# HaiminLuo/svox_t

Measured on AMD Instinct MI355X. Metric: Mrays/s fwd+bwd, 800×800 render, depth-8 SH9 N3Tree, 1→8 MI355X, higher is better.
Workload: dtype f32

## Files before the change

### svox_t_amd/csrc/svoxt_fwd_kernels.h

```cpp
#pragma once

#include <hip/hip_runtime.h>
#include <stdint.h>

#include "svoxt_device.h"
#include "svoxt_lists.h"

#pragma clang fp contract(off)

#ifndef SVOXT_ROLES_CSUM
#define SVOXT_ROLES_CSUM 1
#endif

namespace svoxt {

template <bool N2>
__device__ __forceinline__ uint32_t leaf_slot(const TreeDev& tr, const Ray& r, float t, uint32_t slot) {
    if (slot != 0xffffffffu) return slot;
    Leaf lf;
    locate<N2>(tr, r.ox + t * r.dx, r.oy + t * r.dy, r.oz + t * r.dz, lf);
    return lf.slot;
}

template <int FMT, int C, int BD, bool N2, bool REC, bool XF = false, bool RESUME = false, bool LOBES = false>
__device__ __forceinline__ void render_fwd_ray(const TreeDev& tr, const RaysDev& rays, const Opts& opt, float* __restrict__ out,
                                               const RecLists& L, uint4* __restrict__ aux, const int64_t tid) {
    static_assert(!XF || FMT == FMT_SH, "view rotations only matter for view-dependent formats");
    static_assert(!LOBES || (FMT == FMT_SH && !XF), "lobes stand in for an SH basis");
    static_assert(!(RESUME && REC), "the tail launch does not record");
    constexpr int K = (FMT == FMT_RGBA) ? (C + 1) : (C * BD + 1);
    __shared__ uint2 rstage[REC ? kRecBlock * kBlock : 1];
    __shared__ int32_t ltab[REC ? kMaxRecBlocks : 1];
    __shared__ float4 tstage[(REC && C == 3 && !XF) ? 4 * kBlock : 1];
    if constexpr (REC) rec_tab_init(ltab);
    const int S = L.S;
    int64_t cur_block = 0;
    const int64_t q = ray_of_thread(rays, tid);
    if (q >= rays.Q) return;
    float* o = out + q * (C + 1);
    float t_start = 0.f;
    if constexpr (RESUME) {
        const uint4 a = aux[q];
        if ((a.x & kRecOverflow) == 0u || a.w == kAuxStopped) return;
        t_start = __uint_as_float(a.y);
    }

    Ray r;
    if (!setup_ray(tr, rays, opt, q, r)) {
#pragma unroll
        for (int j = 0; j < C; ++j) o[j] = opt.background_brightness;
        o[C] = 0.f;
        if constexpr (REC) aux[q] = make_uint4(0u, 0u, __float_as_uint(1.f), 0u);
        return;
    }
    int nrec = 0;
    bool over = false;
    float t_resume = 0.f;
    float basis[BD > 0 ? BD : 1];
    float vd[3] = {0.f, 0.f, 0.f};
    if constexpr (FMT == FMT_SH) {
        load_vdir(rays, q, vd);
        if constexpr (LOBES) precalc_lobes<BD>(opt.format, tr, vd[0], vd[1], vd[2], basis);
        else if constexpr (!XF) precalc_basis<BD>(FMT_SH, BD, tr, vd[0], vd[1], vd[2], basis);
    }
    float acc[C];
#pragma unroll
    for (int j = 0; j < C; ++j) acc[j] = 0.f;

    float light = 1.f;
    float t = r.tmin;
    if constexpr (RESUME) {
#pragma unroll
        for (int j = 0; j < C; ++j) acc[j] = o[j];
        light = o[C];
        t = t_start;
    }
    bool stopped = false;
    auto shade = [&](const float (&row)[K], int32_t idx, float delta_t, float t_cur, uint32_t slot) -> bool {
        const float sigma = row[K - 1];
        if (!(sigma > (REC ? 0.f : opt.sigma_thresh))) return false;
        const bool comp = !REC || (sigma > opt.sigma_thresh && !stopped);
        bool recorded = false;
        if constexpr (REC) {
            bool room = nrec < S;
            if (room && (nrec & 7) == 0) {
                cur_block = rec_block_begin(L, ltab, tid >> 6, nrec >> 3);
                room = cur_block >= 0;
            }
            recorded = room;
            if (room) {
                rec_stage_put(rstage, (int)threadIdx.x, L.rec, cur_block, nrec, (uint32_t)idx, delta_t);
                ++nrec;
            } else if (!over) {
                over = true;
                t_resume = t_cur;
            }
        }
        const float att = pexpf(-delta_t * r.delta_scale * sigma);
        const float weight = light * (1.f - att);
        float ex[C];
        if constexpr (FMT == FMT_SH) {
            if constexpr (XF) rotated_sh_basis<BD>(tr, idx, vd, basis);
#pragma unroll
            for (int c = 0; c < C; ++c) {
                ex[c] = pexpf(neg_sh_dot<BD>(basis, row + c * BD));
                if (comp) acc[c] = (float)((double)acc[c] + (double)weight / (1.0 + (double)ex[c]));
            }
        } else {
#pragma unroll
            for (int j = 0; j < C; ++j) {
                ex[j] = pexpf(-row[j]);
                if (comp) acc[j] = (float)((double)acc[j] + (double)weight / (1.0 + (double)ex[j]));
            }
        }
        if constexpr (REC && C == 3 && !XF) {
            if (recorded && L.terms != nullptr) {
                const int k = nrec - 1;
                tstage[(k & 3) * kBlock + threadIdx.x] =
                    make_float4(pexpf(-delta_t * sigma * r.delta_scale), ex[0], ex[1], ex[2]);
                if ((k & 3) == 3) terms_flush(tstage, (int)threadIdx.x, L.terms, cur_block, k);
            }
        }
        if (comp) {
            light *= att;
            if (tr.weight_accum != nullptr) atomicAdd(tr.weight_accum + leaf_slot<N2>(tr, r, t_cur, slot), weight);
            if (light <= opt.stop_thresh) {
                if constexpr (!REC) return true;
                stopped = true;
            }
        }
        return false;
    };
    Sample s;
    bool have = t < r.tmax;
    if (have) march_step<N2>(tr, r, opt.step_size, t, s);
    while (have) {
        float row[K];
        const bool valid = s.valid;
        if (valid) load_row<K>(tr.features + (int64_t)s.idx * K, row);
        const float t_cur = t, delta_t = s.delta_t;
        const int32_t idx = s.idx;
        const uint32_t slot = s.leaf.slot;
        t = march_advance(t, delta_t);
        have = t < r.tmax;
        if (have) march_step<N2>(tr, r, opt.step_size, t, s);
        if (valid && shade(row, idx, delta_t, t_cur, slot)) { stopped = true; break; }
    }
    if (stopped) {
        const float scale = (float)(1.0 / (1.0 - (double)light));
#pragma unroll
        for (int j = 0; j < C; ++j) o[j] = acc[j] * scale;
    } else {
        const float bg = light * opt.background_brightness;
#pragma unroll
        for (int j = 0; j < C; ++j) o[j] = acc[j] + bg;
    }
    o[C] = 1.f - light;
    if constexpr (REC) {
        rec_stage_finish(rstage, (int)threadIdx.x, L.rec, cur_block, nrec);
        if constexpr (C == 3 && !XF) {
            if (L.terms != nullptr && (nrec & 3)) terms_flush(tstage, (int)threadIdx.x, L.terms, cur_block, nrec - 1);
        }
        aux[q] = make_uint4((uint32_t)nrec | (over ? kRecOverflow : 0u), __float_as_uint(t_resume),
                            __float_as_uint(light), 0u);
        if (over) note_overflow(L);
    }
    if constexpr (RESUME) aux[q].z = __float_as_uint(light);
}

template <int FMT, int C, int BD, bool N2, bool REC, bool XF = false, bool RESUME = false, bool LOBES = false>
__global__ void __launch_bounds__(kBlock)
render_fwd_kernel(TreeDev tr, RaysDev rays, Opts opt, float* __restrict__ out,
                  RecLists L, uint4* __restrict__ aux) {
    if constexpr (RESUME) {
        if (no_ray_overflowed(L)) return;
    }
    render_fwd_ray<FMT, C, BD, N2, REC, XF, RESUME, LOBES>(tr, rays, opt, out, L, aux,
                                                           ((int64_t)blockIdx.x + rays.tile0) * kBlock + threadIdx.x);
}

template <bool N2>
__global__ void __launch_bounds__(kBlock)
render_fwd_generic_kernel(TreeDev tr, RaysDev rays, Opts opt, int C, float* __restrict__ out) {
    const int64_t q = ray_of_thread(rays, (int64_t)blockIdx.x * kBlock + threadIdx.x);
    if (q >= rays.Q) return;
    float* o = out + q * (C + 1);
    const int K = tr.K;

    Ray r;
    if (!setup_ray(tr, rays, opt, q, r)) {
        for (int j = 0; j < C; ++j) o[j] = opt.background_brightness;
        o[C] = 0.f;
        return;
    }
    for (int j = 0; j < C; ++j) o[j] = 0.f;
    float basis[25];
    float vd[3];
    load_vdir(rays, q, vd);
    precalc_basis<0>(opt.format, opt.basis_dim, tr, vd[0], vd[1], vd[2], basis);
    float light = 1.f;
    float t = r.tmin;
    while (t < r.tmax) {
        Sample s;
        march_step<N2>(tr, r, opt.step_size, t, s);
        if (s.valid) {
            const float* row = tr.features + (int64_t)s.idx * K;
            const float sigma = row[K - 1];
            if (sigma > opt.sigma_thresh) {
                const float att = pexpf(-s.delta_t * r.delta_scale * sigma);
                const float weight = light * (1.f - att);
                if (tr.xform != nullptr) rotated_basis(tr, opt.format, opt.basis_dim, s.idx, vd, basis);
                if (opt.format != FMT_RGBA) {
                    for (int c = 0; c < C; ++c) {
                        const int off = c * opt.basis_dim;
                        float tmp = 0.f;
                        for (int i = opt.min_comp; i <= opt.max_comp; ++i) tmp += basis[i] * row[off + i];
                        o[c] = (float)((double)o[c] + (double)weight / (1.0 + (double)pexpf(-tmp)));
                    }
                } else {
                    for (int j = 0; j < C; ++j)
                        o[j] = (float)((double)o[j] + (double)weight / (1.0 + (double)pexpf(-row[j])));
                }
                light *= att;
                if (tr.weight_accum != nullptr) atomicAdd(tr.weight_accum + leaf_slot<N2>(tr, r, t, s.leaf.slot), weight);
                if (light <= opt.stop_thresh) {
                    const float scale = (float)(1.0 / (1.0 - (double)light));
                    for (int j = 0; j < C; ++j) o[j] *= scale;
                    o[C] = 1.f - light;
                    return;
                }
            }
        }
        t = march_advance(t, s.delta_t);
    }
    for (int j = 0; j < C; ++j) o[j] += light * opt.background_brightness;
    o[C] = 1.f - light;
}


__global__ void __launch_bounds__(256)
sigma_mask_kernel(const float* __restrict__ features, int64_t M, int K, float thresh, unsigned long long* __restrict__ mask,
                  unsigned mask_blocks = ~0u, uint4* __restrict__ fill = nullptr, int64_t fill_vec = 0) {
    if (blockIdx.x >= mask_blocks) {
        const int64_t i0 = ((int64_t)(blockIdx.x - mask_blocks) * 256 + threadIdx.x) * 4;
#pragma unroll
        for (int j = 0; j < 4; ++j)
            if (i0 + j < fill_vec) fill[i0 + j] = make_uint4(~0u, ~0u, ~0u, ~0u);
        return;
    }
    const int lane = threadIdx.x & 63;
    const int64_t word0 = ((int64_t)blockIdx.x * 4 + (threadIdx.x >> 6)) * 4;
    const int64_t words = (M + 63) / 64;
    float v[4];
#pragma unroll
    for (int j = 0; j < 4; ++j) {
        const int64_t row = (word0 + j) * 64 + lane;
        v[j] = row < M ? features[row * K + (K - 1)] : thresh;
    }
#pragma unroll
    for (int j = 0; j < 4; ++j) {
        const unsigned long long b = __ballot(v[j] > thresh);
        if (lane == j && word0 + j < words) mask[word0 + j] = b;
    }
}

template <int K>
__global__ void __launch_bounds__(256)
exp_table_kernel(const float* __restrict__ features, int64_t M, float thresh, uint8_t* __restrict__ mask_bytes,
                 float* __restrict__ etab) {
    static_assert(K == 8 || K == 16 || K == 32, "row widths with a table");
    constexpr int P = K / 4, RW = 64 / P;
    typedef float v4f __attribute__((ext_vector_type(4)));
    const int64_t t = (int64_t)blockIdx.x * 256 + threadIdx.x;
    const int64_t row = t / P;
    const int part = (int)(t % P);
    bool bit = false;
    if (row < M) {
        const v4f v = __builtin_nontemporal_load(reinterpret_cast<const v4f*>(features) + t);
        v4f e;
        e.x = pexpf(-v.x); e.y = pexpf(-v.y); e.z = pexpf(-v.z);
        if (part == P - 1) { e.w = v.w; bit = v.w > thresh; }
        else e.w = pexpf(-v.w);
        reinterpret_cast<v4f*>(etab)[t] = e;
    }
    const unsigned long long b = __ballot(bit);
    if (mask_bytes != nullptr && (threadIdx.x & 63) == 0 && row < M) {
        uint32_t bits = 0u;
#pragma unroll
        for (int i = 0; i < RW; ++i) bits |= (uint32_t)((b >> (i * P + P - 1)) & 1ull) << i;
        uint8_t* dst = mask_bytes + (row >> 3);
#pragma unroll
        for (int j = 0; j < RW / 8; ++j) dst[j] = (uint8_t)(bits >> (8 * j));
    }
}

template <bool N2, bool STOP, int ACC, bool MASK, bool CSUM = false>
__device__ __forceinline__ uint32_t march_rec_tile(const TreeDev& tr, const RaysDev& rays, const Opts& opt, const RecLists& L,
                                                   uint4* __restrict__ aux, const uint32_t* __restrict__ sigma_mask,
                                                   int64_t tile, uint2* __restrict__ rstage, int32_t* __restrict__ ltab,
                                                   uint32_t* csum = nullptr) {
    static_assert(!(MASK && STOP), "the stop rule needs sigma itself");
    const int lane = (int)(threadIdx.x & 63);
    uint32_t cs = 0u;
    if (csum != nullptr) *csum = 0u;
    rec_tab_init(ltab);
    const int S = L.S;
    int64_t cur_block = 0;
    const int64_t tid = tile * 64 + lane;
    const int64_t q = ray_of_thread(rays, tid);
    if (q >= rays.Q) return 0u;
    Ray r;
    if (!setup_ray(tr, rays, opt, q, r)) {
        aux[q] = make_uint4(0u, 0u, __float_as_uint(1.f), 0u);
        return 0u;
    }
    const int K = tr.K;
    const float* __restrict__ sig_col = tr.features + (K - 1);
    int nrec = 0;
    uint32_t over = 0u;
    float t_resume = 0.f;
    float light = 1.f;
    float t = r.tmin;
    const float kNone = -__builtin_inff();
    float p_sigma = kNone, p_dt = 0.f, p_t = 0.f;
    int32_t p_idx = 0;
    uint32_t p_word = 0u;
    auto pending = [&]() -> bool {
        if constexpr (MASK) return ((p_word >> (p_idx & 31)) & 1u) != 0u;
        else return p_sigma > (STOP ? opt.sigma_thresh : 0.f);
    };
    while (t < r.tmax) {
        Sample s;
        march_step<N2, ACC>(tr, r, opt.step_size, t, s);
        const float t_cur = t;
        t = march_advance(t, s.delta_t);
        bool keep = true;
        if (pending()) {
            bool room = nrec < S;
            if (room && (nrec & 7) == 0) {
                cur_block = rec_block_begin(L, ltab, tid >> 6, nrec >> 3);
                room = cur_block >= 0;
            }
            if (room) {
                rec_stage_put(rstage, lane, L.rec, cur_block, nrec, (uint32_t)p_idx, p_dt);
                if constexpr (CSUM) cs ^= rec_hash(nrec, (uint32_t)p_idx, __float_as_uint(p_dt));
                ++nrec;
                if constexpr (STOP) {
                    light *= pexpf(-p_dt * r.delta_scale * p_sigma);
                    if (light <= opt.stop_thresh) { t = __builtin_inff(); keep = false; }
                }
            } else {
                over = kRecOverflow;
                t_resume = p_t;
                t = __builtin_inff();
                keep = false;
            }
        }
        p_sigma = kNone;
        p_word = 0u;
        if (keep && s.valid) {
            if constexpr (MASK) p_word = sigma_mask[s.idx >> 5];
            else p_sigma = sig_col[(int64_t)s.idx * K];
            p_idx = s.idx;
            p_dt = s.delta_t;
            p_t = t_cur;
        }
    }
    if (pending()) {
        bool room = nrec < S;
        if (room && (nrec & 7) == 0) {
            cur_block = rec_block_begin(L, ltab, tid >> 6, nrec >> 3);
            room = cur_block >= 0;
        }
        if (room) {
            rec_stage_put(rstage, lane, L.rec, cur_block, nrec, (uint32_t)p_idx, p_dt);
            if constexpr (CSUM) cs ^= rec_hash(nrec, (uint32_t)p_idx, __float_as_uint(p_dt));
            ++nrec;
        } else {
            over = kRecOverflow;
            t_resume = p_t;
        }
    }
    rec_stage_finish(rstage, lane, L.rec, cur_block, nrec);
    aux[q] = make_uint4((uint32_t)nrec | over, __float_as_uint(t_resume), __float_as_uint(1.f), 0u);
    if (over != 0u) note_overflow(L);
    if constexpr (CSUM) *csum = cs;
    return (uint32_t)nrec | over;
}

template <bool N2, bool STOP, int ACC, bool MASK = false>
__global__ void __launch_bounds__(kBlock)
march_rec_kernel(TreeDev tr, RaysDev rays, Opts opt, RecLists L, uint4* __restrict__ aux,
                 const uint32_t* __restrict__ sigma_mask = nullptr) {
    __shared__ uint2 rstage[kRecBlock * kBlock];
    __shared__ int32_t ltab[kMaxRecBlocks];
    const int64_t tile = (int64_t)blockIdx.x + rays.tile0;
    march_rec_tile<N2, STOP, ACC, MASK>(tr, rays, opt, L, aux, sigma_mask, tile, rstage, ltab);
}

constexpr int kShadeP = 7;
typedef float shade_v4f __attribute__((ext_vector_type(4)));
template <int FMT, int BD, bool XF, bool STOP, bool WTERMS, bool COH, bool LOBES = false>
__device__ __forceinline__ uint32_t shade_tile_body(const TreeDev& tr, const RaysDev& rays, const Opts& opt, const RecLists& L,
                                                    uint4* __restrict__ aux, float* __restrict__ out, int64_t tile,
                                                    shade_v4f (*terms)[kShadeP][64] ,
                                                    bool stale_test = false, uint32_t* ax_used = nullptr ) {
    constexpr int C = 3, W = 8, P = kShadeP;
    static_assert(P == W - 1, "one wavefront runs along the rays");
    constexpr int K = (FMT == FMT_RGBA) ? (C + 1) : (C * BD + 1);
    constexpr int NB = (FMT == FMT_SH) ? BD : 1;
    typedef shade_v4f v4f;
    const int lane = threadIdx.x & 63, wave = threadIdx.x >> 6;
    const int64_t q = ray_of_thread(rays, tile * 64 + lane);
    const bool inb = q < rays.Q;
    uint32_t a_x = 0u;
    if (inb) a_x = COH ? aux_get_coherent(aux + q).x : aux[q].x;
    int nrec = (int)(a_x & ~kRecOverflow);
    if constexpr (COH) {
        nrec = min(nrec, L.S);
        if (ax_used != nullptr) *ax_used = a_x;
    }
    int maxn = nrec;
    for (int off = 32; off > 0; off >>= 1) maxn = max(maxn, __shfl_xor(maxn, off, 64));
    maxn = __builtin_amdgcn_readfirstlane(maxn);
    const int nround = (maxn + P - 1) / P;
    const int32_t tabreg = rec_tab_reg<COH>(L, tile, lane);
    uint32_t cs = 0u;

    float delta_scale = 0.f;
    float basis[NB];
    float vd[3] = {0.f, 0.f, 0.f};
    if (wave > 0 && nrec > 0) {
        Ray r;
        setup_ray(tr, rays, opt, q, r);
        delta_scale = r.delta_scale;
        if constexpr (FMT == FMT_SH) {
            load_vdir(rays, q, vd);
            if constexpr (LOBES) precalc_lobes<BD>(opt.format, tr, vd[0], vd[1], vd[2], basis);
            else if constexpr (!XF) precalc_basis<BD>(FMT_SH, BD, tr, vd[0], vd[1], vd[2], basis);
        }
    }
    float light = 1.f, acc[C] = {0.f, 0.f, 0.f};
    bool stopped = false;

    for (int rd = 0; rd <= nround; ++rd) {
        if (wave > 0) {
            const int k = rd * P + (wave - 1);
            if (rd < nround && k < nrec) {
                int64_t blk = rec_block_u(L, tabreg, tile, k >> 3);
                if constexpr (COH) blk = min(max(blk, (int64_t)0), L.pool_blocks - 1);
                uint2 e = COH ? rec_get_coherent(L.rec + rec_index_in(blk, lane, k)) : rec_get(L.rec + rec_index_in(blk, lane, k));
                if constexpr (COH) {
                    if (stale_test && k == 0) e.x ^= 1u;
                    if constexpr (SVOXT_ROLES_CSUM != 0) cs ^= rec_hash(k, e.x, e.y);
                    e.x = min(e.x, (uint32_t)(tr.M - 1));
                }
                const int32_t idx = (int32_t)e.x;
                float row[K];
                load_row<K>(tr.features + (int64_t)idx * K, row);
                v4f tv;
                tv.x = pexpf(-__uint_as_float(e.y) * delta_scale * row[K - 1]);
                const bool below = !(row[K - 1] > opt.sigma_thresh);
                if constexpr (FMT == FMT_SH) {
                    if constexpr (XF) rotated_sh_basis<BD>(tr, idx, vd, basis);
                    float ex[C];
#pragma unroll
                    for (int c = 0; c < C; ++c) {
                        ex[c] = pexpf(neg_sh_dot<BD>(basis, row + c * BD));
                    }
                    tv.y = ex[0]; tv.z = ex[1]; tv.w = ex[2];
                } else {
                    tv.y = pexpf(-row[0]); tv.z = pexpf(-row[1]); tv.w = pexpf(-row[2]);
                }
                {
                    v4f tl = tv;
                    tl.x = below ? 1.f : tv.x;
                    terms[rd & 1][wave - 1][lane] = tl;
                }
                if constexpr (WTERMS) {
                    typedef float v4g __attribute__((ext_vector_type(4)));
                    const float att_b = pexpf(-__uint_as_float(e.y) * row[K - 1] * delta_scale);
                    __builtin_nontemporal_store(v4g{att_b, tv.y, tv.z, tv.w},
                                                reinterpret_cast<v4g*>(L.terms + terms_index_pm(blk, lane, k)));
                }
            }
        } else if (rd > 0) {
            const int kb = (rd - 1) * P;
#pragma unroll
            for (int j = 0; j < P; ++j) {
                if (kb + j < nrec && !stopped) {
                    const v4f tv = terms[(rd - 1) & 1][j][lane];
                    const float weight = light * (1.f - tv.x);
                    acc[0] = (float)((double)acc[0] + (double)weight / (1.0 + (double)tv.y));
                    acc[1] = (float)((double)acc[1] + (double)weight / (1.0 + (double)tv.z));
                    acc[2] = (float)((double)acc[2] + (double)weight / (1.0 + (double)tv.w));
                    light *= tv.x;
                    if (light <= opt.stop_thresh) stopped = true;
                }
            }
        }
        lds_barrier();
    }
    if (wave == 0 && inb) {
        uint32_t* aw = reinterpret_cast<uint32_t*>(aux + q);
        float* o = out + q * (C + 1);
        if (stopped) {
            const float scale = (float)(1.0 / (1.0 - (double)light));
#pragma unroll
            for (int j = 0; j < C; ++j) o[j] = acc[j] * scale;
            o[C] = 1.f - light;
            if constexpr (STOP) aw[0] = a_x & ~kRecOverflow;
        } else if (a_x & kRecOverflow) {
#pragma unroll
            for (int j = 0; j < C; ++j) o[j] = acc[j];
            o[C] = light;
        } else {
            const float bg = light * opt.background_brightness;
#pragma unroll
            for (int j = 0; j < C; ++j) o[j] = acc[j] + bg;
            o[C] = 1.f - light;
        }
        aw[2] = __float_as_uint(light);
        if constexpr (!STOP) aw[3] = stopped ? kAuxStopped : 0u;
    }
    return cs;
}

constexpr int kRolePolls = 20000;
constexpr int64_t kTileEmpty = 1 << 30;
__device__ __forceinline__ int my_xcc() { return (int)(__builtin_amdgcn_s_getreg((3 << 11) | 20) & (kRoleXcds - 1)); }
enum { kRoleCtrShaded = 256, kRoleCtrMismatch = 257, kRoleCtrGaveUp = 258, kRoleCtrDropped = 259, kRoleCtrFallback = 260 };
enum { kRoleTestDrop = 1, kRoleTestNoPoll = 2, kRoleTestStale = 4, kRoleAgentFence = 8 };

constexpr int32_t kTileShaded = 0x200;
template <int FMT, int BD, bool XF, bool STOP, bool WTERMS = false, bool LOBES = false>
__global__ void __launch_bounds__(512)
shade_tile_kernel(TreeDev tr, RaysDev rays, Opts opt, RecLists L,
                  uint4* __restrict__ aux, float* __restrict__ out, const int32_t* __restrict__ tile_state = nullptr) {
    static_assert(!LOBES || (FMT == FMT_SH && !XF), "lobes stand in for an SH basis");
    __shared__ shade_v4f terms[2][kShadeP][64];
    const int64_t tile = (int64_t)blockIdx.x + rays.tile0;
    if (tile_state != nullptr && tile_state[tile] == kTileShaded) return;
    shade_tile_body<FMT, BD, XF, STOP, WTERMS, false, LOBES>(tr, rays, opt, L, aux, out, tile, terms);
    if (tile_state != nullptr && threadIdx.x == 0)
        atomicAdd(const_cast<int32_t*>(tile_state) + roles_even(gridDim.x + rays.tile0) + kRoleCtrFallback, 1);
}

template <int FMT, int BD, bool WTERMS, bool LOBES = false, bool XF = false>
__global__ void __launch_bounds__(512)
fwd_finish_kernel(TreeDev tr, RaysDev rays, Opts opt, RecLists L, uint4* __restrict__ aux, float* __restrict__ out,
                  int32_t* __restrict__ tile_state, int ntiles) {
    __shared__ shade_v4f terms[2][kShadeP][64];
    constexpr int CAP = 64;
    __shared__ int32_t s_list[CAP];
    __shared__ int32_t s_n;
    const int run = (ntiles + (int)gridDim.x - 1) / (int)gridDim.x;
    const int t0 = (int)blockIdx.x * run, t1 = min(t0 + run, ntiles);
    if (t0 >= t1) return;
    if (threadIdx.x == 0) s_n = 0;
    __syncthreads();
    for (int i = t0 + (int)threadIdx.x; i < t1; i += 512) {
        if (tile_state[i] != kTileShaded) {
            const int pos = atomicAdd(&s_n, 1);
            if (pos < CAP) s_list[pos] = i;
        }
    }
    __syncthreads();
    const int n = s_n;
    int32_t* const fallback_ctr = tile_state + roles_even(ntiles) + kRoleCtrFallback;
    if (n > CAP) {
        for (int tile = t0; tile < t1; ++tile) {
            if (tile_state[tile] == kTileShaded) continue;
            shade_tile_body<FMT, BD, XF, false, WTERMS, false, LOBES>(tr, rays, opt, L, aux, out, tile, terms);
            if (threadIdx.x == 0) atomicAdd(fallback_ctr, 1);
            __syncthreads();
        }
    } else {
        for (int j = 0; j < n; ++j) {
            shade_tile_body<FMT, BD, XF, false, WTERMS, false, LOBES>(tr, rays, opt, L, aux, out, s_list[j], terms);
            if (threadIdx.x == 0) atomicAdd(fallback_ctr, 1);
            __syncthreads();
        }
    }
    if (no_ray_overflowed(L)) return;
    __syncthreads();
    for (int tile = t0 + (int)(threadIdx.x >> 6); tile < t1; tile += 8)
        render_fwd_ray<FMT, 3, BD, true, false, XF, true, LOBES>(tr, rays, opt, out, L, aux, (int64_t)tile * 64 + (threadIdx.x & 63));
}

__device__ __forceinline__ void publish_tile(int32_t* __restrict__ tile_state, int ntiles, int64_t tile, uint32_t csum,
                                             bool agent_fence) {
    asm volatile("s_waitcnt vmcnt(0)" ::: "memory");
    if (agent_fence) {
        __builtin_amdgcn_fence(__ATOMIC_RELEASE, "agent");
        asm volatile("s_waitcnt vmcnt(0)" ::: "memory");
    }
    if ((threadIdx.x & 63) == 0) {
        const int xcc = my_xcc();
        const int64_t base = roles_even(ntiles);
        int32_t* ctr = tile_state + base + xcc * 32;
        unsigned long long* queue = reinterpret_cast<unsigned long long*>(tile_state + base + 16 * 32) + (int64_t)xcc * ntiles;
        const int pos = __hip_atomic_fetch_add(ctr, 1, __ATOMIC_RELAXED, __HIP_MEMORY_SCOPE_AGENT) + 1;
        __hip_atomic_store(queue + pos, (unsigned long long)(uint32_t)tile | ((unsigned long long)csum << 32), __ATOMIC_RELAXED,
                           __HIP_MEMORY_SCOPE_AGENT);
    }
}
__device__ __forceinline__ unsigned long long pop_tile(int32_t* __restrict__ tile_state, int ntiles, int polls) {
    const int xcc = my_xcc();
    const int64_t base = roles_even(ntiles);
    int32_t* ctr = tile_state + base + xcc * 32;
    unsigned long long* queue = reinterpret_cast<unsigned long long*>(tile_state + base + 16 * 32) + (int64_t)xcc * ntiles;
    unsigned long long ent = ~0ull;
    const int idx = __hip_atomic_fetch_add(ctr + 16, 1, __ATOMIC_RELAXED, __HIP_MEMORY_SCOPE_AGENT) + 1;
    if (idx < ntiles) {
        for (int p = 0; p < polls; ++p) {
            ent = __hip_atomic_load(queue + idx, __ATOMIC_RELAXED, __HIP_MEMORY_SCOPE_AGENT);
            if (ent != ~0ull) break;
            __builtin_amdgcn_s_sleep(16);
        }
    }
    return ent;
}

struct RolesMap {
    int gb, full, gb_last;
    int cnt[8];
};
__host__ __device__ inline int64_t roles_group_of(const RolesMap& m, int b) {
    if (m.gb <= 0) return b;
    const int x = b & 7, s = b >> 3;
    if (s < m.full * m.gb) return ((int64_t)(s / m.gb) * 8 + x) * m.gb + s % m.gb;
    return (int64_t)m.full * 8 * m.gb + (int64_t)x * m.gb_last + (s - m.full * m.gb);
}

template <int FMT, int BD, int ACC, bool WTERMS, bool LOBES = false, bool XF = false>
__global__ void __launch_bounds__(512)
fwd_roles_kernel(TreeDev tr, RaysDev rays, Opts opt, RecLists L, uint4* __restrict__ aux, float* __restrict__ out,
                 const uint32_t* __restrict__ sigma_mask, int32_t* __restrict__ tile_state, int n_march, int ntiles,
                 int tflags , RolesMap map) {
    constexpr int kMarchBytes = 8 * (kRecBlock * 64 * (int)sizeof(uint2) + kMaxRecBlocks * (int)sizeof(int32_t));
    constexpr int kShadeBytes = 2 * kShadeP * 64 * (int)sizeof(shade_v4f);
    __shared__ __attribute__((aligned(16))) unsigned char lds[kMarchBytes > kShadeBytes ? kMarchBytes : kShadeBytes];
    __shared__ unsigned long long s_ent;
    const int wave = threadIdx.x >> 6;
    const bool agent_fence = (tflags & kRoleAgentFence) != 0;
    int32_t* const ctrs = tile_state + roles_even(ntiles);
    if ((int)blockIdx.x < n_march) {
        const int64_t tile = roles_group_of(map, (int)blockIdx.x) * 8 + wave;
        if (tile >= ntiles) return;
        uint2* rstage = reinterpret_cast<uint2*>(lds) + wave * (kRecBlock * 64);
        int32_t* ltab = reinterpret_cast<int32_t*>(lds + 8 * kRecBlock * 64 * sizeof(uint2)) + wave * kMaxRecBlocks;
        __builtin_amdgcn_s_setprio(3);
        uint32_t cs_lane;
        const uint32_t ax = march_rec_tile<true, false, ACC, true, SVOXT_ROLES_CSUM != 0>(tr, rays, opt, L, aux, sigma_mask, tile, rstage, ltab, &cs_lane);
        const bool empty = __ballot(ax != 0u) == 0ull;
        if (empty) {
            const int64_t q = ray_of_thread(rays, tile * 64 + (threadIdx.x & 63));
            if (q < rays.Q) {
                const float light = 1.f, acc = 0.f;
                const float bg = light * opt.background_brightness;
                float* o = out + q * 4;
                o[0] = acc + bg; o[1] = acc + bg; o[2] = acc + bg;
                o[3] = 1.f - light;
            }
            if ((threadIdx.x & 63) == 0) tile_state[tile] = kTileShaded;
        }
        uint32_t csum = 0u;
        if constexpr (SVOXT_ROLES_CSUM != 0) csum = empty ? 0u : tile_checksum(ax != 0u ? cs_lane : 0u, ax, (int)(threadIdx.x & 63));
        publish_tile(tile_state, ntiles, empty ? (tile | kTileEmpty) : tile, csum, agent_fence);
        return;
    }
    const int i = (int)blockIdx.x - n_march, a = i & 7, b = i >> 3;
    if (b >= map.cnt[a]) return;
    if (threadIdx.x == 0) s_ent = pop_tile(tile_state, ntiles, (tflags & kRoleTestNoPoll) ? 1 : kRolePolls);
    __syncthreads();
    const unsigned long long ent = s_ent;
    if (ent == ~0ull) {
        if (threadIdx.x == 0) atomicAdd(ctrs + kRoleCtrGaveUp, 1);
        return;
    }
    const int64_t tile = (int64_t)(uint32_t)ent;
    if (tile >= ntiles) return;
    if ((tflags & kRoleTestDrop) && tile % 3 == 0) {
        if (threadIdx.x == 0) atomicAdd(ctrs + kRoleCtrDropped, 1);
        return;
    }
    if (agent_fence) __builtin_amdgcn_fence(__ATOMIC_ACQUIRE, "agent");
    uint32_t ax = 0u;
    static_assert(!XF || (FMT == FMT_SH && !LOBES && BD <= 9), "view rotations: SH rows");
    const uint32_t part = shade_tile_body<FMT, BD, XF, false, WTERMS, true, LOBES>(
        tr, rays, opt, L, aux, out, tile, reinterpret_cast<shade_v4f (*)[kShadeP][64]>(lds), (tflags & kRoleTestStale) && tile % 5 == 0, &ax);
    uint32_t* s_part = reinterpret_cast<uint32_t*>(lds);
    s_part[threadIdx.x] = part;
    lds_barrier();
    if (wave == 0) {
        const int lane = (int)threadIdx.x;
        uint32_t x = 0u;
#pragma unroll
        for (int w = 0; w < 8; ++w) x ^= s_part[w * 64 + lane];
        const uint32_t c = SVOXT_ROLES_CSUM != 0 ? tile_checksum(ax != 0u ? x : 0u, ax, lane) : (uint32_t)(ent >> 32);
        if (lane == 0) {
        if (c == (uint32_t)(ent >> 32)) {
            tile_state[tile] = kTileShaded;
            atomicAdd(ctrs + kRoleCtrShaded, 1);
        } else {
            atomicAdd(ctrs + kRoleCtrMismatch, 1);
        }
        }
    }
}

#ifndef SVOXT_CHAN_SWIZZLE
#define SVOXT_CHAN_SWIZZLE 1
#endif
template <int K, bool STOP, bool FAST, bool ETAB = false>
__global__ void __launch_bounds__(256)
shade_chan_kernel(TreeDev tr, RaysDev rays, Opts opt, RecLists L,
                  uint4* __restrict__ aux, float* __restrict__ out, int keep_over = 0) {
    static_assert(K == 8 || K == 16 || K == 32, "row widths with a channel-lane instance");
    static_assert(!(ETAB && FAST), "the table holds the exact exponentials");
    constexpr int RPW = 64 / K;
    const int lane = threadIdx.x & 63;
    const int c = lane & (K - 1);
    const int sig_lane = lane | (K - 1);
    constexpr unsigned kRun = (unsigned)(K / 4) * SVOXT_CHAN_SWIZZLE;
    const unsigned b0 = blockIdx.x;
    unsigned wg = b0;
    if (kRun != 0u && (b0 | (8u * kRun - 1u)) < gridDim.x) {
        const unsigned base = b0 & ~(8u * kRun - 1u), x = b0 & 7u, m = (b0 >> 3) & (kRun - 1u);
        wg = base + x * kRun + m;
    }
    const int64_t t = (int64_t)rays.tile0 * 64 + ((int64_t)wg * (blockDim.x >> 6) + (threadIdx.x >> 6)) * RPW + (lane / K);
    const int64_t q = ray_of_thread(rays, t);
    const bool inb = q < rays.Q;
    uint4 a = make_uint4(0u, 0u, 0u, 0u);
    if (inb) a = aux[q];
    const int nrec = (int)(a.x & ~kRecOverflow);
    int maxn = nrec;
    for (int off = 32; off >= K; off >>= 1) maxn = max(maxn, __shfl_xor(maxn, off, 64));
    maxn = __builtin_amdgcn_readfirstlane(maxn);
    float ds = 0.f;
    if (nrec > 0) {
        Ray r;
        setup_ray(tr, rays, opt, q, r);
        ds = r.delta_scale;
    }
    const int32_t tabreg = rec_tab_reg(L, t >> 6, lane);
    float light = 1.f, acc = 0.f;
    bool stopped = false;
    typedef unsigned int v4u __attribute__((ext_vector_type(4)));
    const bool is_sig = c == K - 1;
    const char* __restrict__ col_base = reinterpret_cast<const char*>(ETAB ? tr.etab : tr.features) + 4 * c;
    constexpr float kNegLog2e = -1.44269504088896341f;
    const float sc_mult = is_sig ? ds * kNegLog2e : 0.f, sc_base = is_sig ? 0.f : kNegLog2e;
    for (int kb = 0; kb < maxn; kb += kRecBlock) {
        uint32_t idx[kRecBlock];
        float dt[kRecBlock], ex[kRecBlock];
        const int n_here = nrec - kb;
        const int64_t blk = rec_block_u(L, tabreg, t >> 6, kb >> 3);
        const v4u* line = reinterpret_cast<const v4u*>(L.rec + rec_index_in(blk, t, kb));
#pragma unroll
        for (int j = 0; j < kRecBlock / 2; ++j) {
            const v4u w = __builtin_nontemporal_load(line + j);
            idx[2 * j] = w.x; dt[2 * j] = __uint_as_float(w.y);
            idx[2 * j + 1] = w.z; dt[2 * j + 1] = __uint_as_float(w.w);
        }
        float x[kRecBlock];
#pragma unroll
        for (int j = 0; j < kRecBlock; ++j) {
            const uint32_t row = j < n_here ? idx[j] : 0u;
            x[j] = *reinterpret_cast<const float*>(col_base + (size_t)row * (size_t)(K * 4));
        }
        float att_mine = 1.f;
        if constexpr (ETAB) {
            const int jm = c & (kRecBlock - 1);
            float sg = 0.f, dm = 0.f;
#pragma unroll
            for (int j = 0; j < kRecBlock; ++j) {
                const float sj = __shfl(x[j], sig_lane, 64);
                sg = jm == j ? sj : sg;
                dm = jm == j ? dt[j] : dm;
            }
            att_mine = pexpf((jm < n_here && sg > opt.sigma_thresh) ? -dm * ds * sg : 0.f);
#pragma unroll
            for (int j = 0; j < kRecBlock; ++j) ex[j] = j < n_here ? x[j] : 1.f;
        } else {
#pragma unroll
        for (int j = 0; j < kRecBlock; ++j) {
            if constexpr (FAST) {
                const float e2 = x[j] * __builtin_fmaf(dt[j], sc_mult, sc_base);
                ex[j] = __builtin_amdgcn_exp2f((j < n_here && !(is_sig && !(x[j] > opt.sigma_thresh))) ? e2 : 0.f);
            } else {
                const float arg = is_sig ? ((x[j] > opt.sigma_thresh) ? -dt[j] * ds * x[j] : 0.f) : -x[j];
                ex[j] = pexpf(j < n_here ? arg : 0.f);
            }
        }
        }
#pragma unroll
        for (int j = 0; j < kRecBlock; ++j) {
            const float att = ETAB ? __shfl(att_mine, (lane & ~(K - 1)) + j, 64)
                                   : __shfl(ex[j], sig_lane, 64);
            if (!STOP || !stopped) {
                const float weight = light * (1.f - att);
                if constexpr (FAST) acc = __builtin_fmaf(weight, __builtin_amdgcn_rcpf(1.f + ex[j]), acc);
                else if constexpr (ETAB) acc = (float)((double)acc + div_unit_range((double)weight, 1.0 + (double)ex[j]));
                else acc = (float)((double)acc + (double)weight / (1.0 + (double)ex[j]));
                light *= att;
                if constexpr (STOP) {
                    if (j < n_here && light <= opt.stop_thresh) stopped = true;
                }
            }
        }
    }
    if (!inb) return;
    const bool over = (a.x & kRecOverflow) != 0u && !stopped;
    float v;
    if (c < K - 1) {
        if (stopped) v = acc * (float)(1.0 / (1.0 - (double)light));
        else if (over) v = acc;
        else v = acc + light * opt.background_brightness;
    } else {
        v = over ? light : 1.f - light;
        if (stopped && !keep_over) a.x &= ~kRecOverflow;
        a.z = __float_as_uint(light);
        a.w = (stopped && keep_over) ? kAuxStopped : 0u;
        aux[q] = a;
    }
    out[q * K + c] = v;
}

template <int K, bool N2, bool FAST>
__global__ void __launch_bounds__(256)
tail_chan_kernel(TreeDev tr, RaysDev rays, Opts opt, uint4* __restrict__ aux, float* __restrict__ out, RecLists L) {
    if (no_ray_overflowed(L)) return;
    constexpr int RPW = 64 / K;
    __shared__ int any_over;
    const int lane = threadIdx.x & 63, wave = threadIdx.x >> 6;
    const int64_t tile = (int64_t)blockIdx.x + rays.tile0;
    if (wave == 0) {
        const int64_t q0 = ray_of_thread(rays, tile * 64 + lane);
        bool ov = false;
        if (q0 < rays.Q) { const uint4 a0 = aux[q0]; ov = (a0.x & kRecOverflow) != 0u && a0.w != kAuxStopped; }
        const bool a0 = __any(ov);
        if (lane == 0) any_over = a0 ? 1 : 0;
    }
    __syncthreads();
    if (!any_over) return;
    const int c = lane & (K - 1);
    const int sig_lane = lane | (K - 1);
    for (int grp = wave; grp < 64 / RPW; grp += 4) {
        const int64_t t0 = tile * 64 + grp * RPW + (lane / K);
        const int64_t q = ray_of_thread(rays, t0);
        uint4 a = make_uint4(0u, 0u, 0u, 0u);
        if (q < rays.Q) a = aux[q];
        const bool tail = (a.x & kRecOverflow) != 0u && a.w != kAuxStopped;
        bool alive = tail;
        if (!__any(alive)) continue;
        Ray r;
        float light = 1.f, acc = 0.f, t = 0.f, tmax = -1.f;
        bool stopped = false;
        if (alive) {
            setup_ray(tr, rays, opt, q, r);
            t = __uint_as_float(a.y);
            tmax = r.tmax;
            light = out[q * K + (K - 1)];
            if (c < K - 1) acc = out[q * K + c];
        }
        while (__any(alive && t < tmax)) {
            const bool go = alive && t < tmax;
            float x = 0.f, dt = 0.f;
            bool valid = false;
            if (go) {
                Sample s;
                march_step<N2>(tr, r, opt.step_size, t, s);
                dt = s.delta_t;
                valid = s.valid;
                if (valid) x = tr.features[(int64_t)s.idx * K + c];
                t = march_advance(t, s.delta_t);
            }
            const float sigma = __shfl(x, sig_lane, 64);
            const bool active = go && valid && sigma > opt.sigma_thresh;
            float ex = 1.f;
            if (active) {
                const float arg = c == K - 1 ? -dt * r.delta_scale * x : -x;
                ex = FAST ? nexpf(arg) : pexpf(arg);
            }
            const float att = __shfl(ex, sig_lane, 64);
            if (active) {
                const float weight = light * (1.f - att);
                if constexpr (FAST) acc = __builtin_fmaf(weight, __builtin_amdgcn_rcpf(1.f + ex), acc);
                else acc = (float)((double)acc + (double)weight / (1.0 + (double)ex));
                light *= att;
                if (light <= opt.stop_thresh) { stopped = true; alive = false; }
            }
        }
        if (!tail) continue;
        float v;
        if (c < K - 1) {
            v = stopped ? acc * (float)(1.0 / (1.0 - (double)light)) : acc + light * opt.background_brightness;
        } else {
            v = 1.f - light;
            aux[q].z = __float_as_uint(light);
        }
        out[q * K + c] = v;
    }
}

}
```

Baseline: 1306.

## Stage record blocks into LDS ring buffer with bulk 128-bit loads during shading

```diff
diff --git a/svox_t_amd/csrc/svoxt_fwd_kernels.h b/svox_t_amd/csrc/svoxt_fwd_kernels.h
--- a/svox_t_amd/csrc/svoxt_fwd_kernels.h
+++ b/svox_t_amd/csrc/svoxt_fwd_kernels.h
@@ -400,21 +400,45 @@
 
 constexpr int kShadeP = 7;
 typedef float shade_v4f __attribute__((ext_vector_type(4)));
-template <int FMT, int BD, bool XF, bool STOP, bool WTERMS, bool COH, bool LOBES = false>
+constexpr int kShadeWin = 9, kShadeWinSmall = 6;
+constexpr int kShadeStageRecs = kShadeWin * kRecBlock * 64, kShadeStageRecsSmall = kShadeWinSmall * kRecBlock * 64;
+typedef unsigned int shade_v4u __attribute__((ext_vector_type(4)));
+__device__ __forceinline__ int shade_stage_at(int slot, int kk, int ray) {
+    return (slot * kRecBlock + kk) * 64 + (ray ^ ((kk >> 1) << 3));
+}
+template <bool COH>
+__device__ __forceinline__ shade_v4u shade_stage_load(const uint2* __restrict__ rec, int64_t blk, int c) {
+    const uint2* base = rec + (blk << 9);
+    if constexpr (COH) {
+        const __amdgpu_buffer_rsrc_t rsrc = __builtin_amdgcn_make_buffer_rsrc(const_cast<uint2*>(base), 0, 64 * kRecBlock * 8, 0x00020000);
+        return __builtin_bit_cast(shade_v4u, __builtin_amdgcn_raw_buffer_load_b128(rsrc, c * 16, 0, 16 ));
+    } else {
+        return __builtin_nontemporal_load(reinterpret_cast<const shade_v4u*>(base) + c);
+    }
+}
+__device__ __forceinline__ void shade_stage_store(uint2* __restrict__ stage, int slot, int c, shade_v4u v) {
+    const int ray = c >> 2, kk = (c & 3) * 2;
+    stage[shade_stage_at(slot, kk, ray)] = make_uint2(v.x, v.y);
+    stage[shade_stage_at(slot, kk + 1, ray)] = make_uint2(v.z, v.w);
+}
+template <int FMT, int BD, bool XF, bool STOP, bool WTERMS, bool COH, bool LOBES = false, int NBW = kShadeWin>
 __device__ __forceinline__ uint32_t shade_tile_body(const TreeDev& tr, const RaysDev& rays, const Opts& opt, const RecLists& L,
                                                     uint4* __restrict__ aux, float* __restrict__ out, int64_t tile,
                                                     shade_v4f (*terms)[kShadeP][64] ,
+                                                    uint2* __restrict__ stage ,
                                                     bool stale_test = false, uint32_t* ax_used = nullptr ) {
     constexpr int C = 3, W = 8, P = kShadeP;
+    static_assert(NBW >= 4, "a refilled block is handed over rounds before its first use");
     static_assert(P == W - 1, "one wavefront runs along the rays");
     constexpr int K = (FMT == FMT_RGBA) ? (C + 1) : (C * BD + 1);
     constexpr int NB = (FMT == FMT_SH) ? BD : 1;
     typedef shade_v4f v4f;
-    const int lane = threadIdx.x & 63, wave = threadIdx.x >> 6;
+    const int lane = threadIdx.x & 63, wave = __builtin_amdgcn_readfirstlane(threadIdx.x >> 6);
     const int64_t q = ray_of_thread(rays, tile * 64 + lane);
     const bool inb = q < rays.Q;
     uint32_t a_x = 0u;
     if (inb) a_x = COH ? aux_get_coherent(aux + q).x : aux[q].x;
+    const int32_t tabreg = rec_tab_reg<COH>(L, tile, lane);
     int nrec = (int)(a_x & ~kRecOverflow);
     if constexpr (COH) {
         nrec = min(nrec, L.S);
@@ -424,7 +448,20 @@
     for (int off = 32; off > 0; off >>= 1) maxn = max(maxn, __shfl_xor(maxn, off, 64));
     maxn = __builtin_amdgcn_readfirstlane(maxn);
     const int nround = (maxn + P - 1) / P;
-    const int32_t tabreg = rec_tab_reg<COH>(L, tile, lane);
+    const int need = (maxn + kRecBlock - 1) >> 3;
+    constexpr int NSV = (NBW * 256 + 511) / 512;
+    shade_v4u sv[NSV];
+    auto stage_block = [&](int b ) -> int64_t {
+        int64_t blk = rec_block_u(L, tabreg, tile, b);
+        if constexpr (COH) blk = min(max(blk, (int64_t)0), L.pool_blocks - 1);
+        return blk;
+    };
+    const int nb0 = min(need, NBW);
+#pragma unroll
+    for (int i = 0; i < NSV; ++i) {
+        const int b = 2 * i + (wave >> 2);
+        if (b < nb0) sv[i] = shade_stage_load<COH>(L.rec, stage_block(b), (int)(threadIdx.x & 255));
+    }
     uint32_t cs = 0u;
 
     float delta_scale = 0.f;
@@ -442,14 +479,19 @@
     }
     float light = 1.f, acc[C] = {0.f, 0.f, 0.f};
     bool stopped = false;
+#pragma unroll
+    for (int i = 0; i < NSV; ++i) {
+        const int b = 2 * i + (wave >> 2);
+        if (b < nb0) shade_stage_store(stage, b, (int)(threadIdx.x & 255), sv[i]);
+    }
+    __builtin_amdgcn_s_waitcnt(0x0f70);
+    lds_barrier();
 
     for (int rd = 0; rd <= nround; ++rd) {
         if (wave > 0) {
             const int k = rd * P + (wave - 1);
             if (rd < nround && k < nrec) {
-                int64_t blk = rec_block_u(L, tabreg, tile, k >> 3);
-                if constexpr (COH) blk = min(max(blk, (int64_t)0), L.pool_blocks - 1);
-                uint2 e = COH ? rec_get_coherent(L.rec + rec_index_in(blk, lane, k)) : rec_get(L.rec + rec_index_in(blk, lane, k));
+                uint2 e = stage[shade_stage_at((k >> 3) % NBW, k & 7, lane)];
                 if constexpr (COH) {
                     if (stale_test && k == 0) e.x ^= 1u;
                     if constexpr (SVOXT_ROLES_CSUM != 0) cs ^= rec_hash(k, e.x, e.y);
@@ -481,22 +523,39 @@
                     typedef float v4g __attribute__((ext_vector_type(4)));
                     const float att_b = pexpf(-__uint_as_float(e.y) * row[K - 1] * delta_scale);
                     __builtin_nontemporal_store(v4g{att_b, tv.y, tv.z, tv.w},
-                                                reinterpret_cast<v4g*>(L.terms + terms_index_pm(blk, lane, k)));
+                                                reinterpret_cast<v4g*>(L.terms + terms_index_pm(stage_block(k >> 3), lane, k)));
                 }
             }
         } else if (rd > 0) {
-            const int kb = (rd - 1) * P;
-#pragma unroll
-            for (int j = 0; j < P; ++j) {
-                if (kb + j < nrec && !stopped) {
-                    const v4f tv = terms[(rd - 1) & 1][j][lane];
-                    const float weight = light * (1.f - tv.x);
-                    acc[0] = (float)((double)acc[0] + (double)weight / (1.0 + (double)tv.y));
-                    acc[1] = (float)((double)acc[1] + (double)weight / (1.0 + (double)tv.z));
-                    acc[2] = (float)((double)acc[2] + (double)weight / (1.0 + (double)tv.w));
-                    light *= tv.x;
-                    if (light <= opt.stop_thresh) stopped = true;
+            const int d = (rd * P) >> 3;
+            const bool refill = d > (((rd - 1) * P) >> 3) && d - 1 + NBW < need;
+            auto chain = [&]() {
+                const int kb = (rd - 1) * P;
+#pragma unroll
+                for (int j = 0; j < P; ++j) {
+                    if (kb + j < nrec && !stopped) {
+                        const v4f tv = terms[(rd - 1) & 1][j][lane];
+                        const float weight = light * (1.f - tv.x);
+                        acc[0] = (float)((double)acc[0] + (double)weight / (1.0 + (double)tv.y));
+                        acc[1] = (float)((double)acc[1] + (double)weight / (1.0 + (double)tv.z));
+                        acc[2] = (float)((double)acc[2] + (double)weight / (1.0 + (double)tv.w));
+                        light *= tv.x;
+                        if (light <= opt.stop_thresh) stopped = true;
+                    }
                 }
+            };
+            if (refill) {
+                int rl = lane;
+                asm volatile("" : "+v"(rl));
+                const int64_t blk = stage_block(d - 1 + NBW);
+                shade_v4u rf[4];
+#pragma unroll
+                for (int j = 0; j < 4; ++j) rf[j] = shade_stage_load<COH>(L.rec, blk, j * 64 + rl);
+                chain();
+#pragma unroll
+                for (int j = 0; j < 4; ++j) shade_stage_store(stage, (d - 1) % NBW, j * 64 + rl, rf[j]);
+            } else {
+                chain();
             }
         }
         lds_barrier();
@@ -539,9 +598,10 @@
                   uint4* __restrict__ aux, float* __restrict__ out, const int32_t* __restrict__ tile_state = nullptr) {
     static_assert(!LOBES || (FMT == FMT_SH && !XF), "lobes stand in for an SH basis");
     __shared__ shade_v4f terms[2][kShadeP][64];
+    __shared__ uint2 stage[kShadeStageRecsSmall];
     const int64_t tile = (int64_t)blockIdx.x + rays.tile0;
     if (tile_state != nullptr && tile_state[tile] == kTileShaded) return;
-    shade_tile_body<FMT, BD, XF, STOP, WTERMS, false, LOBES>(tr, rays, opt, L, aux, out, tile, terms);
+    shade_tile_body<FMT, BD, XF, STOP, WTERMS, false, LOBES, kShadeWinSmall>(tr, rays, opt, L, aux, out, tile, terms, stage);
     if (tile_state != nullptr && threadIdx.x == 0)
         atomicAdd(const_cast<int32_t*>(tile_state) + roles_even(gridDim.x + rays.tile0) + kRoleCtrFallback, 1);
 }
@@ -551,6 +611,7 @@
 fwd_finish_kernel(TreeDev tr, RaysDev rays, Opts opt, RecLists L, uint4* __restrict__ aux, float* __restrict__ out,
                   int32_t* __restrict__ tile_state, int ntiles) {
     __shared__ shade_v4f terms[2][kShadeP][64];
+    __shared__ uint2 stage[kShadeStageRecsSmall];
     constexpr int CAP = 64;
     __shared__ int32_t s_list[CAP];
     __shared__ int32_t s_n;
@@ -571,13 +632,13 @@
     if (n > CAP) {
         for (int tile = t0; tile < t1; ++tile) {
             if (tile_state[tile] == kTileShaded) continue;
-            shade_tile_body<FMT, BD, XF, false, WTERMS, false, LOBES>(tr, rays, opt, L, aux, out, tile, terms);
+            shade_tile_body<FMT, BD, XF, false, WTERMS, false, LOBES, kShadeWinSmall>(tr, rays, opt, L, aux, out, tile, terms, stage);
             if (threadIdx.x == 0) atomicAdd(fallback_ctr, 1);
             __syncthreads();
         }
     } else {
         for (int j = 0; j < n; ++j) {
-            shade_tile_body<FMT, BD, XF, false, WTERMS, false, LOBES>(tr, rays, opt, L, aux, out, s_list[j], terms);
+            shade_tile_body<FMT, BD, XF, false, WTERMS, false, LOBES, kShadeWinSmall>(tr, rays, opt, L, aux, out, s_list[j], terms, stage);
             if (threadIdx.x == 0) atomicAdd(fallback_ctr, 1);
             __syncthreads();
         }
@@ -634,12 +695,14 @@
 }
 
 template <int FMT, int BD, int ACC, bool WTERMS, bool LOBES = false, bool XF = false>
-__global__ void __launch_bounds__(512)
+__global__ void __launch_bounds__(512, (BD <= 9 && !XF) ? 6 : 0)
 fwd_roles_kernel(TreeDev tr, RaysDev rays, Opts opt, RecLists L, uint4* __restrict__ aux, float* __restrict__ out,
                  const uint32_t* __restrict__ sigma_mask, int32_t* __restrict__ tile_state, int n_march, int ntiles,
                  int tflags , RolesMap map) {
     constexpr int kMarchBytes = 8 * (kRecBlock * 64 * (int)sizeof(uint2) + kMaxRecBlocks * (int)sizeof(int32_t));
-    constexpr int kShadeBytes = 2 * kShadeP * 64 * (int)sizeof(shade_v4f);
+    constexpr int kTermBytes = 2 * kShadeP * 64 * (int)sizeof(shade_v4f);
+    constexpr int kShadeBytes = kTermBytes + kShadeStageRecs * (int)sizeof(uint2);
+    static_assert(kShadeBytes + 8 <= 53248, "three workgroups per CU: 160 KiB / 3, less the allocation granule");
     __shared__ __attribute__((aligned(16))) unsigned char lds[kMarchBytes > kShadeBytes ? kMarchBytes : kShadeBytes];
     __shared__ unsigned long long s_ent;
     const int wave = threadIdx.x >> 6;
@@ -689,7 +752,7 @@
     uint32_t ax = 0u;
     static_assert(!XF || (FMT == FMT_SH && !LOBES && BD <= 9), "view rotations: SH rows");
     const uint32_t part = shade_tile_body<FMT, BD, XF, false, WTERMS, true, LOBES>(
-        tr, rays, opt, L, aux, out, tile, reinterpret_cast<shade_v4f (*)[kShadeP][64]>(lds), (tflags & kRoleTestStale) && tile % 5 == 0, &ax);
+        tr, rays, opt, L, aux, out, tile, reinterpret_cast<shade_v4f (*)[kShadeP][64]>(lds), reinterpret_cast<uint2*>(lds + kTermBytes), (tflags & kRoleTestStale) && tile % 5 == 0, &ax);
     uint32_t* s_part = reinterpret_cast<uint32_t*>(lds);
     s_part[threadIdx.x] = part;
     lds_barrier();
```

Result: faster. 1328 (median of 6 runs) (+1.7%).
